# raviraj988/3D-POINT-CLOUD-SEGMENTATION-USING-2D-IMG-SEGMENTATION

Measured on AMD Instinct MI355X. Metric: labelled points/sec (10M pts x 64 views) at 1/2/4/8 GPU; % HBM roofline, higher is better.
Workload: dtype f64; 1 GPU; C3: 10000000 points x 64 ring views, 1024x1024 block64 uint8 masks, nclasses=133, threshold=0.5, filter_classes=None; fused project->sample->vote->segment; points_total=10000000, points_per_gpu=10000000, views=64, xyz_storage=f64, cloud_layout=caller order, cell-sorted inside every step (F3D_FUSE_SORT), exchange=none

## Files before the change

3d-point-cloud-segmentation-using-2d-img-segmentation_amd/csrc/f3d_capi.cpp:

```cpp
#include "f3d_ctx.h"

namespace {

void inv3(const double K[9], double o[9]) {
    const double a = K[0], b = K[1], c = K[2], d = K[3], e = K[4], f = K[5], g = K[6], h = K[7], i = K[8];
    const double A = e * i - f * h, B = c * h - b * i, C = b * f - c * e;
    const double D = f * g - d * i, E = a * i - c * g, F = c * d - a * f;
    const double G = d * h - e * g, H = b * g - a * h, I = a * e - b * d;
    const double det = (a * A + b * D) + c * G;
    o[0] = A / det; o[1] = B / det; o[2] = C / det;
    o[3] = D / det; o[4] = E / det; o[5] = F / det;
    o[6] = G / det; o[7] = H / det; o[8] = I / det;
}

struct frustum { double eye[3], lookat[3], normal[4][3]; };

void frustum_of(const double K[9], double w, double h, const double q[4], const double t[3], frustum* fr) {
    double Ki[9];
    inv3(K, Ki);
    const double pix[6][3] = {{0, 0, 0}, {0, 0, 1}, {w, 0, 1}, {w, h, 1}, {0, h, 1}, {w / 2, h / 2, 1}};
    double world[6][3];
    for (int k = 0; k < 6; ++k) {
        f3d_p3 c;
        c.x = (Ki[0] * pix[k][0] + Ki[1] * pix[k][1]) + Ki[2] * pix[k][2];
// ... 426 lines not shown
        return fail(ctx, F3D_ERR_INVALID, "fastpath_audit: bad arguments");
    staging st(ctx);
    const void* dxyz = st.in(xyz, xyz_bytes(dtype, n));
    void* dsorted = st.slot(xyz_bytes(dtype, n));
    int32_t* dperm = (int32_t*)st.slot((size_t)n * 4);
    const f3d_view* dviews = st.in(views, sizeof(f3d_view) * (size_t)nviews);
    void* dstats = st.slot(64);
    st.back(stats, dstats, 32);
    if (st.rc) return st.rc;
    if ((rc = f3d_cloud_sort_cells_dev(ctx, dxyz, dtype, n, dsorted, dperm, ctx->stream))) return rc;
    F3D_HIP(ctx, f3d_launch_fastpath_audit(dsorted, dtype, n, dviews, nviews, w, h, (unsigned long long*)dstats, ctx->stream));
    return st.finish();
}

int f3d_debug_fuse_deferred(f3d_ctx* ctx, void* stream, uint32_t counts[2]) {
    int rc = enter(ctx); if (rc) return rc;
    if (!counts || !ctx->scratch[SLOT_TODO].p) return fail(ctx, F3D_ERR_INVALID, "fuse_deferred: no fused call has run in this context");
    hipStream_t s = pick(ctx, stream);
    F3D_HIP(ctx, hipMemcpyAsync(counts, f3d_fuse_todo::counters(ctx->scratch[SLOT_TODO].p), 8, hipMemcpyDeviceToHost, s));
    F3D_HIP(ctx, hipStreamSynchronize(s));
    return F3D_OK;
}

int f3d_project_vote_argmax(f3d_ctx* ctx, const void* xyz, f3d_dtype dtype, int64_t n, const f3d_view* views, int nviews,
                            const uint8_t* masks, int h, int w, int nclasses, const int32_t* filter, int nfilter,
                            double threshold, int64_t* classes, uint16_t* votes_u16) {
    int rc = enter(ctx); if (rc) return rc;
    if (n < 0 || nviews < 0 || h <= 0 || w <= 0 || nclasses < 0 || !classes || (n > 0 && !xyz) || (nviews > 0 && (!views || !masks)))
        return fail(ctx, F3D_ERR_INVALID, "project_vote_argmax: bad arguments");
    if (n == 0) return F3D_OK;
    staging st(ctx);
    const void* dxyz = st.in(xyz, xyz_bytes(dtype, n));
    const f3d_view* dviews = st.in(views, sizeof(f3d_view) * (size_t)nviews);
    const uint8_t* dmasks = st.in(masks, (size_t)nviews * h * w);
    int64_t* dcls = st.out(classes, (size_t)n * 8);
    uint16_t* dvotes = st.out(votes_u16, (size_t)n * ((size_t)nclasses + 1) * 2);
    const unsigned flags = n >= 65536 ? F3D_FUSE_SORT : 0u;
    if (!st.rc) st.rc = f3d_project_vote_argmax_dev(ctx, dxyz, dtype, n, dviews, nviews, dmasks, h, w, nclasses, filter, nfilter, threshold,
                                                    dcls, dvotes, flags, nullptr, ctx->stream);
    return st.finish(F3D_DEVERR_FUSE);
}

int ensure_table(f3d_ctx* ctx, int64_t hw) {
    size_t want = 1024;
    while (want < (size_t)hw * 2) want <<= 1;
    if (ctx->table_slots < want) {
// ... 2999 lines not shown
```

3d-point-cloud-segmentation-using-2d-img-segmentation_amd/csrc/f3d_fuse.hip:

```cpp
#include <hip/hip_runtime.h>
#include <stdint.h>
#include <stdlib.h>
#include <string.h>
#include "f3d.h"
#include "f3d_math.h"
#include "f3d_kernels.h"
#include "f3d_fuse_blocks.h"
#include "f3d_fuse_deal.h"
#include <cstdlib>

#pragma clang fp contract(off)

#define F3D_NO_PREFILL ((int64_t)0x7fffffffffffffffLL)
#define F3D_PART_MAX_GROUPS 16
#ifndef F3D_MID_DENSE
#define F3D_MID_DENSE 8
#endif
#ifndef F3D_NT_CLASSES
#define F3D_NT_CLASSES 1
#endif
#if defined(F3D_EXP_STORE) && F3D_EXP_STORE == 2
#define F3D_STORE_CLASS(p, v) ((void)(v))
#elif defined(F3D_EXP_STORE) && F3D_EXP_STORE == 3
#define F3D_STORE_CLASS(p, v) (reinterpret_cast<uint8_t*>(classes)[(p) - classes] = (uint8_t)(v))
#elif defined(F3D_EXP_STORE) && F3D_EXP_STORE == 4
#define F3D_STORE_CLASS(p, v) __builtin_nontemporal_store((uint8_t)(v), reinterpret_cast<uint8_t*>(classes) + ((p) - classes))
#elif defined(F3D_EXP_STAMP)
#define F3D_STORE_CLASS(p, v) do { if ((p) - classes >= F3D_STAMP_WORDS) __builtin_nontemporal_store((int64_t)(v), (p)); } while (0)
#elif F3D_NT_CLASSES
#define F3D_STORE_CLASS(p, v) __builtin_nontemporal_store((int64_t)(v), (p))
#else
#define F3D_STORE_CLASS(p, v) (*(p) = (v))
#endif
#define F3D_STAMP_WORDS (4 * 8192)
#if defined(F3D_EXP_STAMP)
#define F3D_STAMP_EXIT() do { if (n >= F3D_STAMP_WORDS && lane == 0) atomicMax(reinterpret_cast<unsigned long long*>(classes) + 4 * blockIdx.x + 3, (unsigned long long)wall_clock64()); } while (0)
// ... 395 lines not shown
#undef F3D_L63
}

#ifndef F3D_VTAB_GLOBAL
#define F3D_VTAB_GLOBAL 0
#endif
#ifndef F3D_FUSE_WAVES
#define F3D_FUSE_WAVES 3
#endif
__global__ __launch_bounds__(F3D_BLOCK) void k_fuse_setup(f3d_setup_args a) { f3d_fuse_setup_block(a, blockIdx.x, gridDim.x, F3D_BLOCK); }

template <typename T, int PPL, bool WRITE_VOTES, bool BIN32, bool WRAP, bool TLDS, bool CARRY>
__global__ __launch_bounds__(F3D_BLOCK, F3D_FUSE_WAVES) void k_fuse(const T* __restrict__ xyz, int64_t n,
                                                     const f3d_view* __restrict__ views, int nviews,
                                                     const uint8_t* __restrict__ cmasks, int H, int W,
                                                     int nclasses, int nfilter, const int* __restrict__ fcls, double threshold,
                                                     int64_t* __restrict__ classes, uint16_t* __restrict__ votes_out,
                                                     int* __restrict__ err, const int32_t* __restrict__ perm, int gather_xyz,
                                                     unsigned int* __restrict__ todo_count, int32_t* __restrict__ todo,
                                                     const f3d_codebook* __restrict__ cb, int cmin, int cmax,
                                                     const float* __restrict__ ctabT, const double* __restrict__ vtabT,
                                                     uint32_t* __restrict__ carry, int chunk_flags, T* __restrict__ xyz_keep,
                                                     unsigned long long* __restrict__ umask, uint32_t* __restrict__ park, int park_slots, int park_stride,
                                                     int64_t prefilled, const f3d_deal deal) {
#if defined(F3D_EXP_STAMP)
    const long long stamp_entry = wall_clock64();
    bool stamp_first = true;
#endif
    const int ncodes = cb->ncodes;
    if (ncodes > cmax || ncodes < cmin) return;
    const int words = (ncodes + 3) >> 2;
    const int hdw = BIN32 ? ncodes : words;
    extern __shared__ uint32_t lds_u32[];
    float* ctab = reinterpret_cast<float*>(lds_u32);
    uint32_t* lutw = TLDS ? lds_u32 + 64 * F3D_CULL_ROW : lds_u32;
    double* vtab = reinterpret_cast<double*>(lutw + F3D_BOOK_DWORDS);
    uint32_t* hist = (TLDS && !F3D_VTAB_GLOBAL) ? lutw + F3D_BOOK_DWORDS + 2 * F3D_VHEAD * 64 : lutw + F3D_BOOK_DWORDS;
    const uint16_t* vmin = (WRAP || nviews > 255) ? nullptr : reinterpret_cast<const uint16_t*>(lutw + 128);
    const uint8_t* lut = reinterpret_cast<const uint8_t*>(lutw);
    const uint8_t* inv = lut + 256;
    const int tid = threadIdx.x, lane = threadIdx.x & 63;
    constexpr int TILE = F3D_BLOCK * PPL;
    const int npts = (int)n;
    const int ntiles = (int)((n + TILE - 1) / TILE);
    const unsigned plane = (unsigned)f3d_coded_plane(H, W);
    const int pitch = f3d_coded_pitch(W);
    const int c_row = 64 * pitch - 64;
    const int ngroups = (nviews + 63) >> 6;
    const float umaxf = (float)(W > H ? W : H), Wf = (float)W, Hf = (float)H;

    const __amdgpu_buffer_rsrc_t cm_rsrc = __builtin_amdgcn_make_buffer_rsrc(const_cast<uint8_t*>(cmasks), 0, (int)((unsigned)nviews * plane), 0x00020000);
#if defined(F3D_EXP_GATHER) && F3D_EXP_GATHER == 1
    auto gather = [&](unsigned off) -> unsigned { return (unsigned)__builtin_amdgcn_raw_buffer_load_b8(cm_rsrc, (int)(off & 63u), 0, 0); };
#elif defined(F3D_EXP_GATHER) && F3D_EXP_GATHER == 2
    auto gather = [&](unsigned off) -> unsigned { return off & 2u; };
#else
    auto gather = [&](unsigned off) -> unsigned { return (unsigned)__builtin_amdgcn_raw_buffer_load_b8(cm_rsrc, (int)off, 0, 0); };
#endif
    auto stage_group = [&](int g) {
        float cv[6]; double vv[4];
#pragma unroll
        for (int r = 0; r < 6; ++r) cv[r] = ctabT[((size_t)g * 24 + (tid >> 6) + 4 * r) * 64 + lane];
#pragma unroll
// ... 119 lines not shown
#pragma unroll
                        for (int b4 = 0; b4 < 4; ++b4) if (4 * wd + b4 < ncodes) hc[(4 * wd + b4) * F3D_BLOCK] = (x >> (8 * b4)) & 0xFFu;
                    } else {
                        hc[wd * F3D_BLOCK] = x;
                    }
                }
            }
        } else {
            for (int wd = 0; wd < hdw; ++wd) { hcol0[wd * F3D_BLOCK] = 0u; if (PPL == 2) hcol1[wd * F3D_BLOCK] = 0u; }
        }
        unsigned nvalid[2] = {0u, 0u};
        unsigned pend[2] = {F3D_CODE_NONE, F3D_CODE_NONE};
        unsigned ccode[2][F3D_CHUNK];
#pragma unroll
        for (int k = 0; k < F3D_CHUNK; ++k) ccode[0][k] = ccode[1][k] = F3D_CODE_NONE;
#if F3D_GATHER_DEPTH == 2
        unsigned ccode2[2][F3D_CHUNK];
#pragma unroll
        for (int k = 0; k < F3D_CHUNK; ++k) ccode2[0][k] = ccode2[1][k] = F3D_CODE_NONE;
#define F3D_OLDEST ccode2
#else
#define F3D_OLDEST ccode
#endif
        auto vote = [&](int q, unsigned b) {
            if (q >= PPL) return;
            if (BIN32) vote_bin32(q ? hcol1 : hcol0, b);
            else vote_coded<WRAP || CARRY>(nvalid[q], q ? hcol1 : hcol0, b);
        };

        for (int g = 0; g < ngroups; ++g) {
            const int vj = 64 * g + lane;
            bool box_out = false, box_in = true, own_image = false;
            float pb0 = 0.f, pb1 = 0.f, pb2 = 0.f, pb3 = 0.f, pb4 = 0.f, pmarg = 0.f;
            unsigned pneed = 0u;
            if (vj < nviews) {
                const float* rowp = TLDS ? ctab + lane * F3D_CULL_ROW : ctabT + (size_t)g * 24 * 64 + lane;
                auto rowf = [&](int f) { return TLDS ? rowp[f] : rowp[f * 64]; };
                const float marg = 2.0f * __builtin_fmaf(rowf(20), ps_box, rowf(21));
                float bmax = 0.f, smax = 0.f, base[F3D_NPLANES];
                unsigned need = 0u;
#pragma unroll
                for (int m = 0; m < F3D_NPLANES; ++m) {
                    const float n0 = rowf(3 * m), n1 = rowf(3 * m + 1), n2 = rowf(3 * m + 2);
                    base[m] = __builtin_fmaf(n0, c0, __builtin_fmaf(n1, c1, __builtin_fmaf(n2, c2, -rowf(15 + m))));
                    const float spread = __builtin_fmaf(fabsf(n0), e0, __builtin_fmaf(fabsf(n1), e1, fabsf(n2) * e2));
                    box_out = box_out | (base[m] + spread < -marg);
                    box_in = box_in & (base[m] - spread > marg);
                    need |= (base[m] - spread > marg) ? 0u : (1u << m);
                    bmax = fmaxf(bmax, fabsf(base[m])); smax = fmaxf(smax, spread);
                }
                pb0 = base[0]; pb1 = base[1]; pb2 = base[2]; pb3 = base[3]; pb4 = base[4];
                pneed = need;
                pmarg = 0.5f * marg + 1.01f * (float)F3D_U24 * (4.0f * bmax + 5.0f * smax);
                own_image = (int)(rowf(22) == Wf) & (int)(rowf(23) == Hf);
            }
            centre_row mine = {0.f, 0.f, 0.f, 0.f, 0.f, 0.f, 0.f, 0.f, 0.f, 0.f, 0.f, 0.f, 0u, 0, 0};
            bool row_ok = false;
            if (vj < nviews && !box_out && wave_any)
                row_ok = centre_precompute((TLDS && !F3D_VTAB_GLOBAL) ? vtab + lane : vtabT + (size_t)g * F3D_VHEAD * 64 + lane, 64, c0, c1, c2, e0, e1, e2, umaxf, pitch, mine);
            mine.obase += (unsigned)vj * plane;
            const unsigned long long valid_m = __ballot(vj < nviews);
            unsigned long long out_m = __ballot(vj < nviews && box_out);
            const unsigned long long in_m = __ballot(vj < nviews && box_in && !box_out && own_image);
            const unsigned long long row_m = __ballot(row_ok);
            if (!wave_any) out_m = valid_m;
            unsigned long long todo_v = valid_m & ~out_m & in_m & row_m;
#if defined(F3D_EXP_SKIP) && (F3D_EXP_SKIP == 1 || F3D_EXP_SKIP == 3)
            todo_v = 0ull;
#endif
            while (todo_v) {
                int cbit[F3D_CHUNK]; unsigned coff[2][F3D_CHUNK];
                bool use[F3D_CHUNK];
                unsigned long long unsm[2][F3D_CHUNK];
#pragma unroll
                for (int k = 0; k < F3D_CHUNK; ++k) {
                    use[k] = todo_v != 0ull;
                    cbit[k] = use[k] ? __builtin_ctzll(todo_v) : (k ? cbit[0] : 0);
                    if (use[k]) todo_v &= todo_v - 1ull;
                }
#pragma unroll
                for (int k = 0; k < F3D_CHUNK; ++k) {
                    const centre_row r = read_row(mine, cbit[k]);
                    int fi0[2], fi1[2]; bool safe[2];
                    project_offset2(r, DX, DY, DZ, fi0, fi1, safe);
#pragma unroll
                    for (int q = 0; q < PPL; ++q) {
                        if (PART) unsm[q][k] = __ballot(act[q] & !safe[q]);
                        else unsure[q] = safe[q] ? unsure[q] : 1u;
                        const unsigned o = r.obase + rel_offset(fi0[q], fi1[q], c_row);
                        coff[q][k] = (safe[q] & use[k]) ? o : 0u;
                    }
                }
#ifndef F3D_NO_VOTE_PIN
// ... 14 lines not shown
                if (PART) {
                    unsigned long long au = 0ull;
#pragma unroll
                    for (int k = 0; k < F3D_CHUNK; ++k) au |= unsm[0][k] | (PPL == 2 ? unsm[1][k] : 0ull);
                    if (__builtin_expect(au != 0ull, 0)) {
                        asm volatile("" ::: "memory");
                        const unsigned long long me = 1ull << lane;
#pragma unroll
                        for (int k = 0; k < F3D_CHUNK; ++k)
#pragma unroll
                            for (int q = 0; q < PPL; ++q) um[q] |= (unsm[q][k] & me) ? (1ull << cbit[k]) : 0ull;
                    }
                }
            }
#pragma unroll
            for (int k = 0; k < F3D_CHUNK; ++k) {
#if F3D_GATHER_DEPTH == 2
                vote(0, ccode2[0][k]); vote(1, ccode2[1][k]);
                ccode2[0][k] = ccode2[1][k] = F3D_CODE_NONE;
#endif
                vote(0, ccode[0][k]); vote(1, ccode[1][k]);
                ccode[0][k] = ccode[1][k] = F3D_CODE_NONE;
            }
            todo_v = valid_m & ~out_m & ~(in_m & row_m);
#if defined(F3D_EXP_SKIP) && F3D_EXP_SKIP == 2
            todo_v = 0ull;
#elif defined(F3D_EXP_SKIP) && F3D_EXP_SKIP == 3
            todo_v = 0ull;
#endif
            while (todo_v) {
                const int bit = __builtin_ctzll(todo_v);
                todo_v &= todo_v - 1ull;
                const int v = 64 * g + bit;
                const f3d_view& vw = views[v];
                float nn[F3D_NPLANES][3];
#pragma unroll
                for (int m = 0; m < F3D_NPLANES; ++m) { nn[m][0] = vw.cull_n32[m][0]; nn[m][1] = vw.cull_n32[m][1]; nn[m][2] = vw.cull_n32[m][2]; }
#pragma unroll
                for (int m = 0; m < F3D_NPLANES; ++m) { asm volatile("" : "+s"(nn[m][0])); asm volatile("" : "+s"(nn[m][1])); asm volatile("" : "+s"(nn[m][2])); }
#define F3D_RL1(x) __int_as_float(__builtin_amdgcn_readlane(__float_as_int(x), bit))
                const float mg = F3D_RL1(pmarg);
                const unsigned need = (unsigned)__builtin_amdgcn_readlane((int)pneed, bit);
                const float* pbs[F3D_NPLANES] = {&pb0, &pb1, &pb2, &pb3, &pb4};
                const bool has_row = (row_m >> bit) & 1ull;
                bool maybe[2] = {true, true}, sure[2] = {true, true};
#pragma unroll
                for (int m = 0; m < F3D_NPLANES; ++m) {
// ... 93 lines not shown
            const bool d = defer[q] | full;
            if (d) {
                const int sl = (PART && slot[q] >= 0) ? slot[q] : (int)atomicAdd(todo_count, 1u);
                full = full | !part_rt | (sl >= park_slots) | !(PART && slot[q] >= 0);
                if (BIN32 && !full && nviews > 255)
                    for (int c = 1; c < ncodes; ++c) full = full | (hc[c * F3D_BLOCK] > 255u);
                todo[sl] = (gather_xyz ? orig[q] : (i0 + 64 * q)) | (full ? (int)0x80000000 : 0);
                if (PART && !full) {
                    uint32_t* pk = park + (size_t)sl * park_stride;
                    for (int wd = 0; wd < words; ++wd) {
                        uint32_t x = 0u;
                        if (BIN32) {
#pragma unroll
                            for (int b4 = 0; b4 < 4; ++b4) if (4 * wd + b4 < ncodes) x |= (hc[(4 * wd + b4) * F3D_BLOCK] & 0xFFu) << (8 * b4);
                        } else {
                            x = hc[wd * F3D_BLOCK];
                        }
                        pk[wd] = wd == 0 ? (x & ~0xFFu) : x;
                    }
                }
            }
            if (bad & !d) atomicOr(err, F3D_DEVERR_FUSE);
        }
        if (jn >= tiles_per_xcd) break;
        j = jn; jn = jnn;
    }
    F3D_STAMP_EXIT();
}

__device__ __forceinline__ void cull_point64(const f3d_view& vw, f3d_p3 p, double pscale, bool& maybe, bool& sure) {
    const double marg = __builtin_fma(vw.cull_rel64, pscale, vw.cull_abs64);
    bool mb = true, sr = true;
#pragma unroll
    for (int m = 0; m < F3D_NPLANES; ++m) {
        const double a = __builtin_fma(vw.plane_n[m][0], p.x, __builtin_fma(vw.plane_n[m][1], p.y,
                         __builtin_fma(vw.plane_n[m][2], p.z, -vw.plane_off[m])));
        mb = mb & (a > -marg);
        sr = sr & (a > marg);
    }
    maybe = mb; sure = sr;
}

__device__ __forceinline__ bool project_fast(const f3d_view& vw, double umax, f3d_p3 p, int W, int H, int& iu, int& iv, bool& unsure) {
    const double d0 = p.x - vw.t[0], d1 = p.y - vw.t[1], d2 = p.z - vw.t[2];
    const double h0 = __builtin_fma(vw.M[0], d0, __builtin_fma(vw.M[1], d1, vw.M[2] * d2));
    const double h1 = __builtin_fma(vw.M[3], d0, __builtin_fma(vw.M[4], d1, vw.M[5] * d2));
    const double h2 = __builtin_fma(vw.M[6], d0, __builtin_fma(vw.M[7], d1, vw.M[8] * d2));
    const double r = rcp_newton(h2);
// ... 432 lines not shown
    const bool fast = j.cmasks != nullptr;
    if (CARRY && (!fast || nviews > 255 || !j.carry || v0 < 0 || v1 <= v0 || v1 > nviews)) return hipErrorInvalidValue;
    const int chunk_flags = CARRY ? ((v0 > 0 ? 1 : 0) | (v1 < nviews ? 2 : 0)) : 0;
    const f3d_view* cviews = j.views_dev + v0;
    const uint8_t* ccm = fast ? j.cmasks + (size_t)v0 * f3d_coded_plane(h, w) : nullptr;
    const int cnv = v1 - v0;
    if (fast && (n > 0x7ffff000LL || (flt.nfilter > 0 && !flt.cls_dev) || (uint64_t)nviews * f3d_coded_plane(h, w) >= (1ull << 32)))
        return hipErrorInvalidValue;
    const dim3 b(F3D_BLOCK), ge(fast ? 512 : grid);
    const int words_max = j.lay.park_stride;
    const size_t lds_small = fuse_lds_bytes(F3D_BIN32_MAX_CODES, 2, cnv <= 64), lds_full = fuse_lds_bytes(words_max, 2, false);
    const fuse_tables tab = fuse_tables_split(j.tables, cnv);
    const size_t lds_exact = exact_lds_bytes(mode, nclasses);
    if (lds_exact > 160 * 1024 || lds_full > 160 * 1024) return hipErrorInvalidValue;
    hipError_t e;
    int64_t prefilled = F3D_NO_PREFILL;
    if (fast && !(chunk_flags & 2)) {
        prefilled = unlabelled_after_remap(nclasses, flt);
        if (prefilled != F3D_NO_PREFILL && !j.filled)
            hipLaunchKernelGGL(k_fill_labels, dim3(f3d_grid_for(n, F3D_BLOCK, 2048)), dim3(F3D_BLOCK), 0, s, j.classes, n, prefilled);
    }
    if (fast) {
        const bool wrap = nviews + 3 * ((nviews + 63) / 64) + 2 > 255;
        const bool one_group = cnv <= 64;
        auto ks = one_group ? k_fuse<T, 2, V, true, false, true, CARRY> : k_fuse<T, 2, V, true, false, false, CARRY>;
        auto km2 = k_fuse<T, 2, V, false, false, true, CARRY>;
        auto km3 = k_fuse<T, 2, V, false, false, false, CARRY>;
        auto kf = km3;
        if (!CARRY && wrap) { km2 = k_fuse<T, 2, V, false, true, true, false>; km3 = kf = k_fuse<T, 2, V, false, true, false, false>; }
        if (!one_group) km2 = km3;
        const size_t lds_large = fuse_lds_bytes(words_max < F3D_PACKED_LARGE_WORDS ? words_max : F3D_PACKED_LARGE_WORDS, 2, false);
        if ((e = raise_lds(ks, lds_small)) != hipSuccess || (e = raise_lds(kf, lds_full > lds_large ? lds_full : lds_large)) != hipSuccess) return e;
        const size_t lds_mid = fuse_lds_bytes(F3D_PACKED_SMALL_WORDS, 2, one_group);
        const int positions = f3d_xcd_list_of((int)((n + 2 * F3D_BLOCK - 1) / (2 * F3D_BLOCK))).positions;
        auto fuse = [&](decltype(ks) kernel, size_t lds, int cmin, int cmax, int per_cu) {
            const f3d_deal deal = f3d_deal_make(positions, fuse_slots_per_xcd(j.occ, (const void*)kernel, lds, per_cu), F3D_FUSE_GRID / 8);
            hipLaunchKernelGGL(kernel, dim3(8 * deal.width[0]), b, lds, s, xyz, n, cviews, cnv, ccm, h, w, nclasses, flt.nfilter, flt.cls_dev, j.threshold,
                               j.classes, j.votes, j.err, j.perm, gather, todo_count, todo, j.cb, cmin, cmax, tab.ctabT, tab.vtabT,
                               j.carry, chunk_flags, (T*)j.xyz_keep, umask, park, j.lay.park_slots, j.lay.park_stride, prefilled, deal);
        };
        fuse(ks, lds_small, 0, F3D_BIN32_MAX_CODES, 4);
        if (nclasses + 3 > F3D_BIN32_MAX_CODES) fuse(km2, lds_mid, F3D_BIN32_MAX_CODES + 1, 4 * F3D_PACKED_SMALL_WORDS, one_group ? 4 : 3);
        if (nclasses + 3 > 4 * F3D_PACKED_SMALL_WORDS) fuse(km3, lds_large, 4 * F3D_PACKED_SMALL_WORDS + 1, 4 * F3D_PACKED_LARGE_WORDS, 3);
        if (nclasses + 3 > 4 * F3D_PACKED_LARGE_WORDS) fuse(kf, lds_full, 4 * F3D_PACKED_LARGE_WORDS + 1, 256, 2);
        if (chunk_flags & 2) return hipGetLastError();
        const bool wide = nviews > 255;
        if (wide && !j.masks) return hipErrorInvalidValue;
        auto km = k_fuse_mid<T, V>;
        const size_t lds_tier2 = mid_lds_bytes(words_max);
        if ((e = raise_lds(km, lds_tier2)) != hipSuccess) return e;
        hipLaunchKernelGGL(km, dim3(1024), b, lds_tier2, s, xyz, todo_count, todo, j.views_dev, nviews, j.cmasks, h, w, nclasses, flt.nfilter,
                           flt.cls_dev, j.threshold, j.classes, j.votes, j.err, j.perm, gather, wide ? todo_count + 2 : (unsigned int*)nullptr,
                           wide ? todo2 : (int32_t*)nullptr, todo2_count, j.cb,
                           (const unsigned long long*)umask, (const uint32_t*)park, j.lay.park_slots, j.lay.park_stride);
        if (!wide) return hipGetLastError();
    }
    const unsigned int* exact_count = fast ? todo_count + 2 : todo2_count;
    const int32_t* exact_list = fast ? todo2 : nullptr;
    auto ke = mode == MODE_HIST8 ? k_fuse_exact<T, MODE_HIST8, V> : k_fuse_exact<T, MODE_HIST16, V>;
    if ((e = raise_lds(ke, lds_exact)) != hipSuccess) return e;
    hipLaunchKernelGGL(ke, ge, b, lds_exact, s, xyz, n, exact_count, exact_list, j.views_dev, nviews, j.masks, h, w, nclasses,
                       flt, j.threshold, j.classes, j.votes, j.err, j.perm, gather);
// ... 66 lines not shown
```

3d-point-cloud-segmentation-using-2d-img-segmentation_amd/csrc/f3d_fuse_blocks.h:

```cpp
#pragma once
#include <hip/hip_runtime.h>
#include <stdint.h>
#include "f3d.h"
#include "f3d_kernels.h"

#define F3D_RIDER_THREADS 512
#ifndef F3D_RIDER_UNROLL
#define F3D_RIDER_UNROLL 6
#endif
#ifndef F3D_RIDER_UNROLL_1
#define F3D_RIDER_UNROLL_1 8
#endif
#ifndef F3D_RIDER_BLOCKS_1
#define F3D_RIDER_BLOCKS_1 256
#endif
#ifndef F3D_RIDER_BLOCKS_2
#define F3D_RIDER_BLOCKS_2 1024
#endif
#ifndef F3D_RIDER_BLOCKS_FILL
#define F3D_RIDER_BLOCKS_FILL 512
#endif
#ifndef F3D_RIDER_SMALL_POINTS
#define F3D_RIDER_SMALL_POINTS (512 * 8192)
#endif
// ... 101 lines not shown
    __syncthreads();
    if (threadIdx.x < 256) {
        const unsigned long long m = __ballot(seen[threadIdx.x] != 0);
        if ((threadIdx.x & 63) == 0) { blkset[threadIdx.x >> 5] = (unsigned)m; blkset[(threadIdx.x >> 5) + 1] = (unsigned)(m >> 32); }
    }
    __syncthreads();
    f3d_presence_publish(blkset, cb);
}

__device__ __forceinline__ void f3d_threshold_table(f3d_codebook* __restrict__ cb, double threshold) {
    const int t = threadIdx.x;
    if (t >= 256) return;
    int lo = 0, hi = t + 1;
    while (lo < hi) {
        const int mid = (lo + hi) >> 1;
        if ((double)mid / (double)t < threshold) lo = mid + 1; else hi = mid;
    }
    cb->cmin[t] = (uint16_t)lo;
}

__device__ __forceinline__ void f3d_code_lut_block(f3d_codebook* __restrict__ cb, int nclasses, int book, const f3d_filter_args& flt) {
    __shared__ unsigned pres[8];
    __shared__ int first_of[256];
    __shared__ unsigned long long wb[4];
    const unsigned l = threadIdx.x;
    const bool act = l < 256u;
    if (l < 8) { pres[l] = book == 1 ? cb->presence[l] : 0xFFFFFFFFu; cb->presence[l] = 0u; }
    if (act) { first_of[l] = -1; cb->inv[l] = 0; }
    __syncthreads();
    if (book == 2) {
        if (l == 0)
            for (int k = flt.nfilter - 1; k >= 0; --k) { const int f = f3d_filter_at(flt, k); if (f >= 0 && f < 256) first_of[f] = k; }
        __syncthreads();
        if (!act) return;
        const bool listed = first_of[l] >= 0 && (int)l <= nclasses;
        int rank = 0;
        for (unsigned j = 0; j < l; ++j) rank += (first_of[j] >= 0 && (int)j <= nclasses) ? 1 : 0;
        int distinct = 0;
        for (unsigned j = 0; j < 256; ++j) distinct += (first_of[j] >= 0 && (int)j <= nclasses) ? 1 : 0;
        const unsigned code = (int)l > nclasses ? F3D_CODE_BAD : (listed ? 3u + (unsigned)rank : F3D_CODE_OTHER);
        cb->lut[l] = (uint8_t)code;
        if (listed) cb->inv[code] = (uint8_t)l;
        if (l == 0) { cb->ncodes = 3 + distinct; cb->words = (3 + distinct + 3) >> 2; cb->book = 2; }
        return;
    }
    const bool pv = act && (int)l <= nclasses && ((pres[(l >> 5) & 7u] >> (l & 31u)) & 1u);
    const unsigned long long bal = __ballot(pv);
    if (act && (l & 63u) == 0u) wb[l >> 6] = bal;
    __syncthreads();
    if (!act) return;
    int K = 0, below = __popcll(bal & ((1ull << (l & 63u)) - 1ull));
    for (unsigned w = 0; w < 4; ++w) { const int c = __popcll(wb[w]); K += c; below += (w < (l >> 6)) ? c : 0; }
    unsigned code;
    if ((int)l > nclasses) code = F3D_CODE_BAD;
    else if (pv) code = (unsigned)(K + 1 - below);
    else code = F3D_CODE_NONE;
    cb->lut[l] = (uint8_t)code;
    if (code >= 2u) cb->inv[code] = (uint8_t)l;
    if (l == 0) { cb->ncodes = K + 2; cb->words = (K + 2 + 3) >> 2; cb->book = book; }
}

template <bool VEC>
__device__ __forceinline__ void f3d_code_masks_block(const uint8_t* __restrict__ src, uint8_t* __restrict__ dst, int V, int H, int W,
                                                     const f3d_codebook* __restrict__ cb, int blk, int nblk, int nthr) {
    __shared__ uint32_t lut_w[64];
    if (threadIdx.x < 64) lut_w[threadIdx.x] = reinterpret_cast<const uint32_t*>(cb->lut)[threadIdx.x];
    __syncthreads();
    const uint8_t* lut = reinterpret_cast<const uint8_t*>(lut_w);
    const int tw = f3d_coded_pitch(W), th = ((H + 7) >> 3) + 2;
    const int64_t per_view = (int64_t)th * tw * 8;
    const int64_t total = per_view * V;
    const size_t tplane = f3d_coded_plane(H, W);
    for (int64_t k = (int64_t)blk * nthr + threadIdx.x; k < total; k += (int64_t)nblk * nthr) {
        const int64_t v = k / per_view; const int64_t r = k - v * per_view;
        uint64_t out = 0;
        const int tile = (int)(r >> 3), ry = (int)(r & 7);
        const int ty = tile / tw, tx = tile - ty * tw;
        const int y = (ty - 1) * 8 + ry, x0 = (tx - 1) * 8;
        if (y >= 0 && y < H && x0 >= 0 && x0 < W) {
            const uint8_t* row = src + (size_t)v * H * W + (size_t)y * W + x0;
            if (VEC) {
                const uint64_t x = *reinterpret_cast<const uint64_t*>(row);
// ... 97 lines not shown
```

3d-point-cloud-segmentation-using-2d-img-segmentation_amd/f3d/__init__.py:

```python
import ctypes as C
import os
from pathlib import Path

import numpy as np

from f3d.tensors import depth_code, dtype_code, host_csr, index_code

__all__ = ['F3DError', 'F3DUnavailable', 'Context', 'default_context', 'library', 'library_path',
           'views_build', 'frustum_data', 'quat_inverse', 'VIEW_DOUBLES', 'F64', 'F32', 'FUSE_SORT', 'FUSE_GATHER']

F64, F32 = 0, 1
FUSE_SORT, FUSE_GATHER = 2, 4
OK, ERR_INVALID, ERR_HIP, ERR_INDEX, ERR_ZERO_QUAT, ERR_NOMEM = 0, -1, -2, -3, -4, -5
VIEW_DOUBLES = 88
OBB_DOUBLES = 15
MAX_OBB = 4096
OBB_OK, OBB_FEW, OBB_DEFERRED = 0, 1, 2
NORM_PLAIN, NORM_FMA, NORM_HOST = 0, 1, 2
NORMALS_MAX_NN = 64
QUAD_OK, QUAD_HORIZONTAL, QUAD_NO_CANDIDATE = 0, 1, 2
QUADS_MAX_INST = 65535
I64, I32 = 0, 1
FEAT_F16, FEAT_F32 = 0, 1
FEAT_MAX_D = 4096
# ... 60 lines not shown
        'f3d_ctx_set_strict': (i32, [vp, i32]),
        'f3d_ctx_alloc_count': (C.c_longlong, [vp]),
        'f3d_quat_inverse': (i32, [vp, vp]),
        'f3d_frustum_data': (i32, [vp, dbl, dbl, vp, vp, i32, vp, vp, vp]),
        'f3d_views_build': (i32, [vp, dbl, dbl, vp, vp, i32, dbl, vp]),
        'f3d_rotate_f64': (i32, [vp, vp, i64, vp, vp]),
        'f3d_rotate_f64_dev': (i32, [vp, vp, i64, vp, vp, vp]),
        'f3d_points2pixel_f64': (i32, [vp, vp, i64, vp, vp, vp, vp]),
        'f3d_points2pixel_dev': (i32, [vp, vp, i32, i64, vp, vp, vp, vp, vp]),
        'f3d_inside_polyhedra_f64': (i32, [vp, vp, i64, vp, vp, i32, vp]),
        'f3d_inside_polyhedra_dev': (i32, [vp, vp, i32, i64, vp, vp, i32, vp, vp]),
        'f3d_project_view_f64': (i32, [vp, vp, i64, vp, vp, vp]),
        'f3d_project_view_dev': (i32, [vp, vp, i32, i64, vp, vp, vp, vp]),
        'f3d_project_vote_argmax': (i32, [vp, vp, i32, i64, vp, i32, vp, i32, i32, i32, vp, i32, dbl, vp, vp]),
        'f3d_project_vote_argmax_dev': (i32, [vp, vp, i32, i64, vp, i32, vp, i32, i32, i32, vp, i32, dbl, vp, vp, C.c_uint, vp, vp]),
        'f3d_mask_presence_dev': (i32, [vp, vp, i32, i32, i32, vp, vp]),
        'f3d_fuse_chunked_begin_dev': (i32, [vp, vp, i64, i32, i32, i32, i32, vp, i32, vp]),
        'f3d_fuse_chunk_dev': (i32, [vp, vp, i32, i64, vp, i32, i32, i32, vp, i32, i32, i32, vp, i32, dbl, vp, C.c_uint, vp, vp]),
        'f3d_coded_plane_bytes': (C.c_size_t, [i32, i32]),
        'f3d_code_planes_dev': (i32, [vp, vp, i32, i32, i32, vp, vp]),
        'f3d_fuse_chunk_coded_dev': (i32, [vp, vp, i32, i64, vp, i32, i32, i32, vp, i32, i32, i32, vp, i32, dbl, vp, C.c_uint, vp, vp]),
        'f3d_debug_fastpath_audit': (i32, [vp, vp, i32, i64, vp, i32, i32, i32, vp]),
        'f3d_debug_fuse_deferred': (i32, [vp, vp, vp]),
        'f3d_cloud_sort_cells_dev': (i32, [vp, vp, i32, i64, vp, vp, vp]),
        'f3d_take_device_error': (i32, [vp, vp]),
        'f3d_vote_uv2pt': (i32, [vp, vp, vp, i64, vp, i64, i32]),
        'f3d_vote_uv2pt_dev': (i32, [vp, vp, vp, i64, vp, i64, i32, vp]),
        'f3d_vote_uv2pt_batch': (i32, [vp, vp, vp, i64, i32, i32, vp, i64, i32]),
        'f3d_vote_uv2pt_batch_dev': (i32, [vp, vp, vp, i64, i32, i32, vp, i64, i32, vp]),
        'f3d_segment_votes': (i32, [vp, vp, i64, i32, i32, dbl, vp, i32, vp]),
        'f3d_segment_votes_dev': (i32, [vp, vp, i64, i32, i32, dbl, vp, i32, vp, vp]),
        'f3d_segment_votes_lastcol': (i32, [vp, vp, i64, i32, i32, dbl, vp, i32, vp]),
        'f3d_segment_votes_lastcol_dev': (i32, [vp, vp, i64, i32, i32, dbl, vp, i32, vp, vp]),
        'f3d_point_vote_frames': (i32, [vp, vp, i32, i64, vp, i32, vp, i64, i64, dbl, vp, i32]),
        'f3d_point_vote_frames_dev': (i32, [vp, vp, i32, i64, vp, i32, vp, i64, i64, dbl, vp, i32, vp]),
        'f3d_ctx_reserve_point_vote': (i32, [vp, i64, i32]),
        'f3d_render_lookups': (i32, [vp, vp, i32, i64, vp, i32, i32, i32, i32, vp, vp]),
        'f3d_render_lookups_dev': (i32, [vp, vp, i32, i64, vp, i32, i32, i32, i32, vp, vp, vp]),
        'f3d_vote_visible': (i32, [vp, vp, i32, i64, vp, i32, vp, i32, i32, i32, dbl, vp, i32, i32]),
        'f3d_vote_visible_dev': (i32, [vp, vp, i32, i64, vp, i32, vp, i32, i32, i32, dbl, vp, i32, i32, vp]),
        'f3d_ctx_reserve_render': (i32, [vp, i64, i32, i32, i32]),
        'f3d_debug_render_counts': (i32, [vp, vp, i32, i64, vp, i32, i32, i32, i32, vp, vp, vp]),
        'f3d_render_mesh_lookups': (i32, [vp, vp, i32, i64, vp, i32, i64, vp, i32, i32, i32, dbl, vp, vp, vp]),
        'f3d_render_mesh_lookups_dev': (i32, [vp, vp, i32, i64, vp, i32, i64, vp, i32, i32, i32, dbl, vp, vp, vp, vp]),
        'f3d_vote_faces': (i32, [vp, vp, i32, i64, vp, i32, i64, vp, i32, vp, i32, i32, dbl, vp, i32, i32]),
        'f3d_vote_faces_dev': (i32, [vp, vp, i32, i64, vp, i32, i64, vp, i32, vp, i32, i32, dbl, vp, i32, i32, vp]),
# ... 1363 lines not shown
        k = _knn_k(k)
        self._check(self._lib.f3d_transfer_labels_dev(self._h, data_ptr, int(data_dtype), int(m), labels_ptr, queries_ptr, int(query_dtype),
                                                      int(n), k, float(radius), int(fill), out_ptr, support_ptr, stream))

    def rotate_dev(self, xyz_ptr, n, q_wxyz, out_ptr, stream=None):
        q = _f64(q_wxyz, (4,))
        self._check(self._lib.f3d_rotate_f64_dev(self._h, xyz_ptr, n, _ptr(q), out_ptr, stream))

    def cloud_sort_cells_dev(self, xyz_ptr, dtype, n, sorted_ptr, perm_ptr, stream=None):
        self._check(self._lib.f3d_cloud_sort_cells_dev(self._h, xyz_ptr, dtype, n, sorted_ptr, perm_ptr, stream))

    def fastpath_audit(self, points, views, w=1024, h=1024):
        p, dt = _xyz(points)
        v = _f64(views)
        stats = np.zeros(4, np.uint64)
        self._check(self._lib.f3d_debug_fastpath_audit(self._h, _ptr(p), dt, len(p), _ptr(v), len(v), int(w), int(h), _ptr(stats)))
        return tuple(int(x) for x in stats)

    def fuse_deferred(self, stream=None):
        c = np.zeros(2, np.uint32)
        self._check(self._lib.f3d_debug_fuse_deferred(self._h, stream, _ptr(c)))
        return int(c[0]), int(c[1])

    def flood_order_dev(self, classes_ptr, n, offsets_ptr, neighbours_ptr, instance_classes, root_ptr, order_ptr, coffs_ptr, flags_ptr,
                        stream=None):
        inst = np.ascontiguousarray(np.asarray(instance_classes).reshape(-1), dtype=np.int64)
        stats = np.zeros(4, np.int64)
        self._check(self._lib.f3d_flood_order_dev(self._h, classes_ptr, int(n), offsets_ptr, neighbours_ptr, _ptr(inst), len(inst), root_ptr,
                                                  order_ptr, coffs_ptr, flags_ptr, _ptr(stats), stream))
        return _flood_stats(stats)

    def color_segment_dev(self, colors_ptr, dtype, n, offsets_ptr, neighbours_ptr, ids_ptr, seeds_ptr, nseeds, threshold, neutral_ids=(0,),
                          max_level=10, accepted_ptr=None, stream=None):
        thr = _threshold3(threshold)
        neu = np.ascontiguousarray(np.asarray(list(neutral_ids)).reshape(-1), dtype=np.int64)
        self._check(self._lib.f3d_color_segment_dev(self._h, colors_ptr, int(dtype), int(n), offsets_ptr, neighbours_ptr, ids_ptr, seeds_ptr,
                                                    int(nseeds), _ptr(thr), _ptr(neu), len(neu), int(max_level), accepted_ptr, stream))

    def region_grow_dev(self, values_ptr, dtype, nchan, n, offsets_ptr, neighbours_ptr, seeds_ptr, nseeds, sma0, npts0, threshold, max_level,
                        cluster_ptr, count_ptr, seeds_given=False, stream=None):
        sma, thr = _grow_params(int(nchan), sma0, threshold)
        self._check(self._lib.f3d_region_grow_dev(self._h, values_ptr, int(dtype), int(nchan), int(n), offsets_ptr, neighbours_ptr, seeds_ptr,
                                                  int(nseeds), _ptr(sma), int(npts0), int(bool(seeds_given)), _ptr(thr), int(max_level),
                                                  cluster_ptr, count_ptr, stream))

    def plane_distance_dev(self, points_ptr, n, plane_point, normal, out_ptr, stream=None):
# ... 321 lines not shown
```

include/f3d.h:

```cpp
#ifndef F3D_H
#define F3D_H

#include <stddef.h>
#include <stdint.h>

#ifdef __cplusplus
extern "C" {
#endif

#define F3D_VERSION 100
#define F3D_MAX_FILTER 512
#define F3D_NPLANES 5

typedef enum f3d_status {
    F3D_OK = 0,
    F3D_ERR_INVALID = -1,
    F3D_ERR_HIP = -2,
    F3D_ERR_INDEX = -3,
    F3D_ERR_ZERO_QUAT = -4,
    F3D_ERR_NOMEM = -5
} f3d_status;

typedef enum f3d_dtype {
    F3D_F64 = 0,
// ... 77 lines not shown
#define F3D_FUSE_GATHER  4u
int f3d_project_vote_argmax_dev(f3d_ctx* ctx, const void* xyz, f3d_dtype dtype, int64_t n,
                                const f3d_view* views_dev , int nviews,
                                const uint8_t* masks, int h, int w,
                                int nclasses, const int32_t* filter , int nfilter,
                                double threshold, int64_t* classes, uint16_t* votes_u16,
                                unsigned flags, const int32_t* perm, void* stream);
int f3d_mask_presence_dev(f3d_ctx* ctx, const uint8_t* masks, int nviews, int h, int w, uint8_t* present256, void* stream);
int f3d_fuse_chunked_begin_dev(f3d_ctx* ctx, const uint8_t* present256, int64_t n, int nviews, int h, int w, int nclasses,
                               const int32_t* filter , int nfilter, void* stream);
int f3d_fuse_chunk_dev(f3d_ctx* ctx, const void* xyz, f3d_dtype dtype, int64_t n, const f3d_view* views_dev, int nviews,
                       int v_begin, int v_end, const uint8_t* masks , int h, int w, int nclasses,
                       const int32_t* filter , int nfilter, double threshold, int64_t* classes,
                       unsigned flags, const int32_t* perm, void* stream);
size_t f3d_coded_plane_bytes(int h, int w);
int f3d_code_planes_dev(f3d_ctx* ctx, const uint8_t* masks, int nplanes, int h, int w, uint8_t* coded, void* stream);
int f3d_fuse_chunk_coded_dev(f3d_ctx* ctx, const void* xyz, f3d_dtype dtype, int64_t n, const f3d_view* views_dev, int nviews,
                             int v_begin, int v_end, const uint8_t* coded , int h, int w,
                             int nclasses, const int32_t* filter , int nfilter, double threshold, int64_t* classes,
                             unsigned flags, const int32_t* perm, void* stream);
int f3d_debug_fastpath_audit(f3d_ctx* ctx, const void* xyz, f3d_dtype dtype, int64_t n,
                             const f3d_view* views, int nviews, int w, int h, uint64_t stats[4]);
int f3d_debug_fuse_deferred(f3d_ctx* ctx, void* stream, uint32_t counts[2]);
int f3d_cloud_sort_cells_dev(f3d_ctx* ctx, const void* xyz, f3d_dtype dtype, int64_t n,
                             void* sorted_xyz, int32_t* perm, void* stream);
int f3d_take_device_error(f3d_ctx* ctx, void* stream);

int f3d_vote_uv2pt(f3d_ctx* ctx, const int32_t* uv2pt, const uint8_t* mask, int64_t hw,
                   double* votes, int64_t npts, int ncols);
int f3d_vote_uv2pt_dev(f3d_ctx* ctx, const int32_t* uv2pt, const uint8_t* mask, int64_t hw,
                       double* votes, int64_t npts, int ncols, void* stream);

int f3d_vote_uv2pt_batch(f3d_ctx* ctx, const int32_t* luts, const uint8_t* masks, int64_t nframes, int h, int w,
                         double* votes, int64_t npts, int ncols);
int f3d_vote_uv2pt_batch_dev(f3d_ctx* ctx, const int32_t* luts, const uint8_t* masks, int64_t nframes, int h, int w,
                             double* votes, int64_t npts, int ncols, void* stream);

int f3d_segment_votes(f3d_ctx* ctx, const double* votes, int64_t npts, int ncols, int nclasses,
                      double threshold, const int32_t* filter, int nfilter, int64_t* classes);
int f3d_segment_votes_dev(f3d_ctx* ctx, const double* votes, int64_t npts, int ncols, int nclasses,
                          double threshold, const int32_t* filter , int nfilter,
                          int64_t* classes, void* stream);

int f3d_segment_votes_lastcol(f3d_ctx* ctx, const double* votes, int64_t npts, int ncols, int nclasses,
                              double threshold, const int32_t* filter, int nfilter, int64_t* classes);
int f3d_segment_votes_lastcol_dev(f3d_ctx* ctx, const double* votes, int64_t npts, int ncols, int nclasses,
// ... 467 lines not shown
```

Measured before the change: 11.89 billion points/s.

## Exit per-wave view loop early once every point is provably unlabelled

Adds an early-decision check inside the fused project/vote kernel. At one or two checkpoints in the last view group, each wave scans its class histograms and uses a bound on the remaining views to test whether every live point can no longer reach the threshold. If so, the wave skips the remaining views. The check applies only when no filter, votes output, carry or wrap is used and the codebook has no out-of-range classes. A debug counter and API report how often waves exit early. The cost is extra histogram scans, an LDS reduction and an atomic per block, which add overhead when waves rarely decide early.

```diff
diff --git a/3d-point-cloud-segmentation-using-2d-img-segmentation_amd/csrc/f3d_capi.cpp b/3d-point-cloud-segmentation-using-2d-img-segmentation_amd/csrc/f3d_capi.cpp
--- a/3d-point-cloud-segmentation-using-2d-img-segmentation_amd/csrc/f3d_capi.cpp
+++ b/3d-point-cloud-segmentation-using-2d-img-segmentation_amd/csrc/f3d_capi.cpp
@@ -472,6 +472,15 @@
     return F3D_OK;
 }
 
+int f3d_debug_fuse_decided(f3d_ctx* ctx, void* stream, uint32_t* count) {
+    int rc = enter(ctx); if (rc) return rc;
+    if (!count || !ctx->scratch[SLOT_TODO].p) return fail(ctx, F3D_ERR_INVALID, "fuse_decided: no fused call has run in this context");
+    hipStream_t s = pick(ctx, stream);
+    F3D_HIP(ctx, hipMemcpyAsync(count, f3d_fuse_todo::counters(ctx->scratch[SLOT_TODO].p) + 3, 4, hipMemcpyDeviceToHost, s));
+    F3D_HIP(ctx, hipStreamSynchronize(s));
+    return F3D_OK;
+}
+
 int f3d_project_vote_argmax(f3d_ctx* ctx, const void* xyz, f3d_dtype dtype, int64_t n, const f3d_view* views, int nviews,
                             const uint8_t* masks, int h, int w, int nclasses, const int32_t* filter, int nfilter,
                             double threshold, int64_t* classes, uint16_t* votes_u16) {
diff --git a/3d-point-cloud-segmentation-using-2d-img-segmentation_amd/csrc/f3d_fuse.hip b/3d-point-cloud-segmentation-using-2d-img-segmentation_amd/csrc/f3d_fuse.hip
--- a/3d-point-cloud-segmentation-using-2d-img-segmentation_amd/csrc/f3d_fuse.hip
+++ b/3d-point-cloud-segmentation-using-2d-img-segmentation_amd/csrc/f3d_fuse.hip
@@ -7,11 +7,20 @@
 #include "f3d_kernels.h"
 #include "f3d_fuse_blocks.h"
 #include "f3d_fuse_deal.h"
+#include "f3d_fuse_decide.h"
 #include <cstdlib>
 
 #pragma clang fp contract(off)
 
 #define F3D_NO_PREFILL ((int64_t)0x7fffffffffffffffLL)
+#ifndef F3D_DECIDE_FIRST
+#define F3D_DECIDE_FIRST 2
+#define F3D_DECIDE_SECOND 1
+#endif
+#ifndef F3D_DECIDE_MIN_MIXED
+#define F3D_DECIDE_MIN_MIXED 2
+#endif
+#define F3D_DECIDE_MIN_VIEWS 8
 #define F3D_PART_MAX_GROUPS 16
 #ifndef F3D_MID_DENSE
 #define F3D_MID_DENSE 8
@@ -453,7 +462,7 @@
                                                      const float* __restrict__ ctabT, const double* __restrict__ vtabT,
                                                      uint32_t* __restrict__ carry, int chunk_flags, T* __restrict__ xyz_keep,
                                                      unsigned long long* __restrict__ umask, uint32_t* __restrict__ park, int park_slots, int park_stride,
-                                                     int64_t prefilled, const f3d_deal deal) {
+                                                     int64_t prefilled, int decide, const f3d_deal deal) {
 #if defined(F3D_EXP_STAMP)
     const long long stamp_entry = wall_clock64();
     bool stamp_first = true;
@@ -470,6 +479,9 @@
     const uint16_t* vmin = (WRAP || nviews > 255) ? nullptr : reinterpret_cast<const uint16_t*>(lutw + 128);
     const uint8_t* lut = reinterpret_cast<const uint8_t*>(lutw);
     const uint8_t* inv = lut + 256;
+    const bool dec_wave = TLDS && !WRITE_VOTES && !CARRY && !WRAP && decide != 0 && vmin != nullptr && cb->pad != 0 &&
+                          (BIN32 || words <= F3D_PACKED_SMALL_WORDS);
+    unsigned n_early = 0u;
     const int tid = threadIdx.x, lane = threadIdx.x & 63;
     constexpr int TILE = F3D_BLOCK * PPL;
     const int npts = (int)n;
@@ -635,6 +647,24 @@
 #else
 #define F3D_OLDEST ccode
 #endif
+        auto scan_bins = [&](const uint32_t* hc, unsigned& lead, unsigned& cast) {
+            if (BIN32) {
+                lead = 0u; cast = hc[F3D_BLOCK];
+                for (int c = 2; c < ncodes; ++c) { const unsigned nc = hc[c * F3D_BLOCK]; cast += nc; lead = lead > nc ? lead : nc; }
+            } else {
+                const unsigned x0 = hc[0];
+                const unsigned c2 = (x0 >> 16) & 0xFFu, c3 = x0 >> 24;
+                cast = ((x0 >> 8) & 0xFFu) + c2 + c3; lead = c2 > c3 ? c2 : c3;
+                for (int wd = 1; wd < words; ++wd) {
+                    const unsigned x = hc[wd * F3D_BLOCK];
+                    cast = __builtin_amdgcn_sad_u8(x, 0u, cast);
+                    const unsigned m01 = (x & 0xFFu) > ((x >> 8) & 0xFFu) ? (x & 0xFFu) : ((x >> 8) & 0xFFu);
+                    const unsigned m23 = ((x >> 16) & 0xFFu) > (x >> 24) ? ((x >> 16) & 0xFFu) : (x >> 24);
+                    lead = lead > m01 ? lead : m01; lead = lead > m23 ? lead : m23;
+                }
+            }
+        };
+        bool left_early = false;
         auto vote = [&](int q, unsigned b) {
             if (q >= PPL) return;
             if (BIN32) vote_bin32(q ? hcol1 : hcol0, b);
@@ -681,7 +711,28 @@
 #if defined(F3D_EXP_SKIP) && (F3D_EXP_SKIP == 1 || F3D_EXP_SKIP == 3)
             todo_v = 0ull;
 #endif
+            const bool chk_on = dec_wave && g == ngroups - 1;
+            const int nwhole = chk_on ? __builtin_popcountll(todo_v) : 0;
+            const unsigned nmixed = (unsigned)__builtin_popcountll(valid_m & ~out_m & ~(in_m & row_m));
+            const unsigned nlater = nmixed + (unsigned)(F3D_CHUNK * F3D_GATHER_DEPTH) + (g > 0 ? 1u : 0u);
+            auto wave_decided = [&](unsigned rout) {
+                bool ok = true;
+#pragma unroll
+                for (int q = 0; q < PPL; ++q) {
+                    unsigned lead, cast;
+                    scan_bins(q ? hcol1 : hcol0, lead, cast);
+                    const bool dq = act[q] & (slot[q] < 0) & (unsure[q] == 0u) &
+                                    f3d_decided_unlabelled(lead, cast, rout + (unsigned)__builtin_popcountll(um[q]), vmin);
+                    ok = ok & (dq | !live[q]);
+                }
+                return (bool)__all(ok);
+            };
+            int chk_at = nwhole >= F3D_DECIDE_MIN_VIEWS ? (nwhole * F3D_DECIDE_FIRST) >> 3 : -1;
             while (todo_v) {
+                if (chk_on && __builtin_popcountll(todo_v) <= chk_at) {
+                    chk_at = chk_at > ((nwhole * F3D_DECIDE_SECOND) >> 3) ? (nwhole * F3D_DECIDE_SECOND) >> 3 : -1;
+                    if (wave_decided((unsigned)__builtin_popcountll(todo_v) + nlater)) { left_early = true; break; }
+                }
                 int cbit[F3D_CHUNK]; unsigned coff[2][F3D_CHUNK];
                 bool use[F3D_CHUNK];
                 unsigned long long unsm[2][F3D_CHUNK];
@@ -742,7 +793,8 @@
                 vote(0, ccode[0][k]); vote(1, ccode[1][k]);
                 ccode[0][k] = ccode[1][k] = F3D_CODE_NONE;
             }
-            todo_v = valid_m & ~out_m & ~(in_m & row_m);
+            if (chk_on && !left_early && nmixed >= F3D_DECIDE_MIN_MIXED && wave_decided(nmixed + (g > 0 ? 1u : 0u))) left_early = true;
+            todo_v = left_early ? 0ull : valid_m & ~out_m & ~(in_m & row_m);
 #if defined(F3D_EXP_SKIP) && F3D_EXP_SKIP == 2
             todo_v = 0ull;
 #elif defined(F3D_EXP_SKIP) && F3D_EXP_SKIP == 3
@@ -882,8 +934,18 @@
             }
             if (bad & !d) atomicOr(err, F3D_DEVERR_FUSE);
         }
+        n_early += left_early ? 1u : 0u;
         if (jn >= tiles_per_xcd) break;
         j = jn; jn = jnn;
+    }
+    static_assert(F3D_BLOCK == 256, "the counter is summed over four waves");
+    if (dec_wave) {
+        if (lane == 0) hcol0[0] = n_early;
+        __syncthreads();
+        if (tid == 0) {
+            const unsigned total = (hist[0] + hist[64]) + (hist[128] + hist[192]);
+            if (total) atomicAdd(todo_count + 3, total);
+        }
     }
     F3D_STAMP_EXIT();
 }
@@ -1362,6 +1424,7 @@
     }
     if (fast) {
         const bool wrap = nviews + 3 * ((nviews + 63) / 64) + 2 > 255;
+        const int decide = (!V && !CARRY && !wrap && cnv <= 64 && flt.nfilter == 0 && j.threshold > 0.0) ? 1 : 0;
         const bool one_group = cnv <= 64;
         auto ks = one_group ? k_fuse<T, 2, V, true, false, true, CARRY> : k_fuse<T, 2, V, true, false, false, CARRY>;
         auto km2 = k_fuse<T, 2, V, false, false, true, CARRY>;
@@ -1377,7 +1440,7 @@
             const f3d_deal deal = f3d_deal_make(positions, fuse_slots_per_xcd(j.occ, (const void*)kernel, lds, per_cu), F3D_FUSE_GRID / 8);
             hipLaunchKernelGGL(kernel, dim3(8 * deal.width[0]), b, lds, s, xyz, n, cviews, cnv, ccm, h, w, nclasses, flt.nfilter, flt.cls_dev, j.threshold,
                                j.classes, j.votes, j.err, j.perm, gather, todo_count, todo, j.cb, cmin, cmax, tab.ctabT, tab.vtabT,
-                               j.carry, chunk_flags, (T*)j.xyz_keep, umask, park, j.lay.park_slots, j.lay.park_stride, prefilled, deal);
+                               j.carry, chunk_flags, (T*)j.xyz_keep, umask, park, j.lay.park_slots, j.lay.park_stride, prefilled, decide, deal);
         };
         fuse(ks, lds_small, 0, F3D_BIN32_MAX_CODES, 4);
         if (nclasses + 3 > F3D_BIN32_MAX_CODES) fuse(km2, lds_mid, F3D_BIN32_MAX_CODES + 1, 4 * F3D_PACKED_SMALL_WORDS, one_group ? 4 : 3);
diff --git a/3d-point-cloud-segmentation-using-2d-img-segmentation_amd/csrc/f3d_fuse_blocks.h b/3d-point-cloud-segmentation-using-2d-img-segmentation_amd/csrc/f3d_fuse_blocks.h
--- a/3d-point-cloud-segmentation-using-2d-img-segmentation_amd/csrc/f3d_fuse_blocks.h
+++ b/3d-point-cloud-segmentation-using-2d-img-segmentation_amd/csrc/f3d_fuse_blocks.h
@@ -147,7 +147,7 @@
 __device__ __forceinline__ void f3d_code_lut_block(f3d_codebook* __restrict__ cb, int nclasses, int book, const f3d_filter_args& flt) {
     __shared__ unsigned pres[8];
     __shared__ int first_of[256];
-    __shared__ unsigned long long wb[4];
+    __shared__ unsigned long long wb[4], wr[4];
     const unsigned l = threadIdx.x;
     const bool act = l < 256u;
     if (l < 8) { pres[l] = book == 1 ? cb->presence[l] : 0xFFFFFFFFu; cb->presence[l] = 0u; }
@@ -166,12 +166,13 @@
         const unsigned code = (int)l > nclasses ? F3D_CODE_BAD : (listed ? 3u + (unsigned)rank : F3D_CODE_OTHER);
         cb->lut[l] = (uint8_t)code;
         if (listed) cb->inv[code] = (uint8_t)l;
-        if (l == 0) { cb->ncodes = 3 + distinct; cb->words = (3 + distinct + 3) >> 2; cb->book = 2; }
+        if (l == 0) { cb->ncodes = 3 + distinct; cb->words = (3 + distinct + 3) >> 2; cb->book = 2; cb->pad = 0; }
         return;
     }
     const bool pv = act && (int)l <= nclasses && ((pres[(l >> 5) & 7u] >> (l & 31u)) & 1u);
-    const unsigned long long bal = __ballot(pv);
-    if (act && (l & 63u) == 0u) wb[l >> 6] = bal;
+    const bool pr = act && (int)l > nclasses && ((pres[(l >> 5) & 7u] >> (l & 31u)) & 1u);
+    const unsigned long long bal = __ballot(pv), balr = __ballot(pr);
+    if (act && (l & 63u) == 0u) { wb[l >> 6] = bal; wr[l >> 6] = balr; }
     __syncthreads();
     if (!act) return;
     int K = 0, below = __popcll(bal & ((1ull << (l & 63u)) - 1ull));
@@ -182,7 +183,7 @@
     else code = F3D_CODE_NONE;
     cb->lut[l] = (uint8_t)code;
     if (code >= 2u) cb->inv[code] = (uint8_t)l;
-    if (l == 0) { cb->ncodes = K + 2; cb->words = (K + 2 + 3) >> 2; cb->book = book; }
+    if (l == 0) { cb->ncodes = K + 2; cb->words = (K + 2 + 3) >> 2; cb->book = book; cb->pad = (book == 1 && !(wr[0] | wr[1] | wr[2] | wr[3])) ? 1 : 0; }
 }
 
 template <bool VEC>
diff --git a/3d-point-cloud-segmentation-using-2d-img-segmentation_amd/csrc/f3d_fuse_decide.h b/3d-point-cloud-segmentation-using-2d-img-segmentation_amd/csrc/f3d_fuse_decide.h
--- /dev/null
+++ b/3d-point-cloud-segmentation-using-2d-img-segmentation_amd/csrc/f3d_fuse_decide.h
@@ -0,0 +1,16 @@
+#pragma once
+#include <stdint.h>
+
+#ifndef __host__
+#define __host__
+#define __device__
+#endif
+
+#define F3D_DECIDE_MAX_TOTAL 255
+
+__host__ __device__ inline bool f3d_decided_unlabelled(unsigned b, unsigned s, unsigned R, const uint16_t* cmin) {
+    const unsigned t = s + R, w = b + R;
+    if (t == 0u || w == 0u) return true;
+    if (t > (unsigned)F3D_DECIDE_MAX_TOTAL) return false;
+    return w < (unsigned)cmin[t];
+}
diff --git a/3d-point-cloud-segmentation-using-2d-img-segmentation_amd/f3d/__init__.py b/3d-point-cloud-segmentation-using-2d-img-segmentation_amd/f3d/__init__.py
--- a/3d-point-cloud-segmentation-using-2d-img-segmentation_amd/f3d/__init__.py
+++ b/3d-point-cloud-segmentation-using-2d-img-segmentation_amd/f3d/__init__.py
@@ -106,6 +106,7 @@
         'f3d_fuse_chunk_coded_dev': (i32, [vp, vp, i32, i64, vp, i32, i32, i32, vp, i32, i32, i32, vp, i32, dbl, vp, C.c_uint, vp, vp]),
         'f3d_debug_fastpath_audit': (i32, [vp, vp, i32, i64, vp, i32, i32, i32, vp]),
         'f3d_debug_fuse_deferred': (i32, [vp, vp, vp]),
+        'f3d_debug_fuse_decided': (i32, [vp, vp, vp]),
         'f3d_cloud_sort_cells_dev': (i32, [vp, vp, i32, i64, vp, vp, vp]),
         'f3d_take_device_error': (i32, [vp, vp]),
         'f3d_vote_uv2pt': (i32, [vp, vp, vp, i64, vp, i64, i32]),
@@ -1515,6 +1516,11 @@
         self._check(self._lib.f3d_debug_fuse_deferred(self._h, stream, _ptr(c)))
         return int(c[0]), int(c[1])
 
+    def fuse_decided(self, stream=None):
+        c = np.zeros(1, np.uint32)
+        self._check(self._lib.f3d_debug_fuse_decided(self._h, stream, _ptr(c)))
+        return int(c[0])
+
     def flood_order_dev(self, classes_ptr, n, offsets_ptr, neighbours_ptr, instance_classes, root_ptr, order_ptr, coffs_ptr, flags_ptr,
                         stream=None):
         inst = np.ascontiguousarray(np.asarray(instance_classes).reshape(-1), dtype=np.int64)
diff --git a/include/f3d.h b/include/f3d.h
--- a/include/f3d.h
+++ b/include/f3d.h
@@ -123,6 +123,7 @@
 int f3d_debug_fastpath_audit(f3d_ctx* ctx, const void* xyz, f3d_dtype dtype, int64_t n,
                              const f3d_view* views, int nviews, int w, int h, uint64_t stats[4]);
 int f3d_debug_fuse_deferred(f3d_ctx* ctx, void* stream, uint32_t counts[2]);
+int f3d_debug_fuse_decided(f3d_ctx* ctx, void* stream, uint32_t* count);
 int f3d_cloud_sort_cells_dev(f3d_ctx* ctx, const void* xyz, f3d_dtype dtype, int64_t n,
                              void* sorted_xyz, int32_t* perm, void* stream);
 int f3d_take_device_error(f3d_ctx* ctx, void* stream);
```

Measured after the change: 12.51 billion points/s, median of 6. 5.2% higher.
